# microsoft/singleshotpose

Hardware: AMD Instinct MI355X
Metric: images/sec (fwd+bwd) yolo-pose 416x416 bs=64/GPU (higher is better)
Workload: dtype f32; 1 GPU; cfg/yolo-pose.cfg train step (zero_grad+fwd+RegionLoss+bwd+grad all-reduce+SGD), 416x416, batch 64/GPU, random-init weights, 1 label/image; global_batch=64, parallelism=dp1

## Files before the change

### include/ssp_hip.h

```cpp
#ifndef SSP_HIP_H
#define SSP_HIP_H
#include <stdint.h>

#ifdef __cplusplus
extern "C" {
#endif

const char* ssp_last_error(void);
int ssp_abi_version(void);
int ssp_set_option(const char* name, int value);


int ssp_conv_fwd(const float* in, const float* wt, float* out, const float* bias, float* stats, int B, int H, int W,
                 int Cin, int Cout, int ldin, int ldout, int R, int accumulate, int plan, float* workspace,
                 int64_t workspace_floats, void* stream);
int ssp_conv_fwd_affine(const float* in, const float* wt, float* out, const float* scale, const float* shift,
                        float slope, int B, int H, int W, int Cin, int Cout, int ldin, int ldout, int R, int plan,
                        float* workspace, int64_t workspace_floats, void* stream);
int ssp_conv_stats_tile_m(int B, int H, int W, int Cin, int Cout, int R, int plan);
int ssp_conv_stats_tiles(int B, int H, int W, int Cin, int Cout, int R, int plan);
int64_t ssp_conv_stats_floats(int B, int H, int W, int Cin, int Cout, int R, int plan);
int ssp_conv_plan_wino_tile(int plan);
int64_t ssp_conv_wino_tiles(int B, int H, int W, int tile);
int ssp_wino_filter_transform_t(const float* w9, float* U, int rows, int K, int tile, void* stream);
// ... 73 lines not shown
                            const float* shift, const float* mean, const float* invstd, int C, int B, int H, int W,
                            float slope, int training, float* partial, int npartial, int zero_after, float* dgamma,
                            float* dbeta, float* c1, float* c2, void* stream);
int ssp_bn_act_bwd_affine(const float* x, int ldx, const float* g, int ldg, float* dx, int lddx, const float* scale,
                          const float* shift, const float* mean, const float* invstd, int C, int B, int H, int W, int pool,
                          float slope, void* stream);
int ssp_bn_bwd_finalize(float* partial, int npartial, int C, int64_t npix, int training, int zero_after, float* dgamma,
                        float* dbeta, float* c1, float* c2, void* stream);
int ssp_colsum(const float* g, int ldg, int64_t M, int C, float* out, void* stream);

int ssp_first_tile_pixels(void);
int ssp_first_groups(int B, int H, int W);
int ssp_first_fwd_stats(const float* x, const float* wt, float* stats, int B, int H, int W, void* stream);
int ssp_first_fwd_apply(const float* x, const float* wt, const float* scale, const float* shift, float slope, float* out,
                        int ldo, int B, int H, int W, void* stream);
int ssp_first_conv_raw(const float* x, const float* wt, float* raw, int ldraw, int B, int H, int W, void* stream);
int ssp_first_bwd_reduce(const float* x, const float* wt, const float* g, int ldg, const float* scale, const float* shift,
                         const float* mean, const float* invstd, float slope, float* partial, int B, int H, int W,
                         void* stream);
int ssp_first_bwd_wgrad(const float* x, const float* wt, const float* g, int ldg, const float* scale, const float* shift,
                        const float* mean, const float* invstd, const float* c1, const float* c2, float slope, float* dw,
                        float* workspace, int64_t workspace_floats, int B, int H, int W, void* stream);
int64_t ssp_first_wgrad_workspace_floats(int B, int H, int W);
int ssp_first_bwd_dgrad(const float* x, const float* wt, const float* g, int ldg, const float* scale, const float* shift,
                        const float* mean, const float* invstd, const float* c1, const float* c2, float slope, float* dx,
                        int B, int H, int W, void* stream);

int ssp_sgd_step(float* param, const float* grad, float* momentum_buf, int64_t n, float lr, float momentum,
                 float dampening, float weight_decay, int nesterov, int first_step, void* stream);
#define SSP_SGD_MAX_TUPLES 16
int ssp_sgd_step_table(float* param, const float* grad, float* momentum_buf, int64_t param_floats, int64_t grad_floats,
                       int64_t momentum_floats, const int64_t* table_dev, const int64_t* table_host, int nseg,
                       const float* hyper, int ntuple, void* stream);

int ssp_nchw_to_nhwc(const float* src, float* dst, int B, int C, int H, int W, int Cpad, int ld, void* stream);
int ssp_nhwc_to_nchw(const float* src, float* dst, int B, int C, int H, int W, int ld, void* stream);
int ssp_u8hwc_to_nhwc(const unsigned char* src, float* dst, int B, int H, int W, int C, int Cpad, int ld, void* stream);
typedef struct SspResampleDesc {
  const void* src;
  void* dst;
  const void* bounds;
  const void* kk;
  const void* img;
  const void* mask;
  const void* lut;
  int src_w, src_h, src_pitch;
// ... 82 lines not shown
```

### singleshotpose_amd/_lib.py

```python
import ctypes
import os
from ctypes import c_char_p, c_double, c_float, c_int, c_int64, c_void_p

_HERE = os.path.dirname(os.path.abspath(__file__))
LIB_PATH = os.environ.get("SSP_HIP_LIB") or os.path.join(_HERE, "libssp_hip.so")


class SspError(RuntimeError):
    pass


_lib = None

P = c_void_p
I = c_int
F = c_float
L = c_int64

_SIGS = {
    "ssp_abi_version": [],
    "ssp_set_option": [c_char_p, I],
    "ssp_conv_fwd": [P, P, P, P, P, I, I, I, I, I, I, I, I, I, I, P, L, P],
    "ssp_conv_fwd_affine": [P, P, P, P, P, F, I, I, I, I, I, I, I, I, I, P, L, P],
    "ssp_conv_stats_tile_m": [I, I, I, I, I, I, I],
# ... 21 lines not shown
    "ssp_conv_wgrad": [P, P, P, I, I, I, I, I, I, I, I, P],
    "ssp_conv_wgrad_route": [I, I, I, I, I, I, I, I],
    "ssp_conv_wgrad_wino": [P, P, P, I, I, I, I, I, I, I, P, L, P],
    "ssp_conv_wgrad_wino_workspace_floats": [I, I, I, I, I],
    "ssp_conv_wgrad_wino_t": [P, P, P, I, I, I, I, I, I, I, I, P, L, P],
    "ssp_conv_wgrad_wino_workspace_floats_t": [I, I, I, I, I, I],
    "ssp_bn_fwd_finalize": [P, I, I, I, I, P, P, P, P, F, F, P, P, P, P, P],
    "ssp_bn_eval_prepare": [I, P, P, P, P, F, P, P, P, P, P],
    "ssp_bn_act_fwd": [P, I, P, I, P, P, I, I, I, I, I, F, P],
    "ssp_bn_bwd_blocks": [],
    "ssp_bn_act_bwd": [P, I, P, I, P, I, P, P, P, P, I, I, I, I, I, F, I, P, P, P, P, P, P],
    "ssp_bn_act_bwd_affine": [P, I, P, I, P, I, P, P, P, P, I, I, I, I, I, F, P],
    "ssp_bn_bwd_finalize": [P, I, I, L, I, I, P, P, P, P, P],
    "ssp_first_tile_pixels": [],
    "ssp_first_groups": [I, I, I],
    "ssp_first_fwd_stats": [P, P, P, I, I, I, P],
    "ssp_first_fwd_apply": [P, P, P, P, F, P, I, I, I, I, P],
    "ssp_first_conv_raw": [P, P, P, I, I, I, I, P],
    "ssp_first_bwd_reduce": [P, P, P, I, P, P, P, P, F, P, I, I, I, P],
    "ssp_first_bwd_wgrad": [P, P, P, I, P, P, P, P, P, P, F, P, P, L, I, I, I, P],
    "ssp_first_bwd_dgrad": [P, P, P, I, P, P, P, P, P, P, F, P, I, I, I, P],
    "ssp_wino_input_transform_t": [P, I, P, I, I, I, I, I, P],
    "ssp_first_wgrad_workspace_floats": [I, I, I],
    "ssp_colsum": [P, I, L, I, P, P],
    "ssp_pose_errors": [P, I, P, P, P, I, I, P, P],
    "ssp_pts_diameter": [P, I, P, P, P],
    "ssp_pose_errors_models": [P, P, P, I, P, P, P, I, I, P, P],
    "ssp_adds_workspace_doubles": [I, I],
    "ssp_adds_errors": [P, P, P, I, I, P, P, I, P, P, L, P],
    "ssp_sgd_step": [P, P, P, L, F, F, F, F, I, I, P],
    "ssp_sgd_step_table": [P, P, P, L, L, L, P, P, I, P, I, P],
    "ssp_nchw_to_nhwc": [P, P, I, I, I, I, I, I, P],
    "ssp_nhwc_to_nchw": [P, P, I, I, I, I, I, P],
    "ssp_u8hwc_to_nhwc": [P, P, I, I, I, I, I, I, P],
    "ssp_resample_u8": [P, I, I, I, I, P],
    "ssp_distort_u8": [P, P, L, P, I, P],
    "ssp_composite_u8": [P, I, L, P],
    "ssp_repack_fwd": [P, P, I, I, I, I, P],
    "ssp_repack_dgrad": [P, P, I, I, I, I, P],
    "ssp_repack_dgrad_packed": [P, P, I, I, I, I, P],
    "ssp_unpack_grad": [P, P, I, I, I, I, P],
    "ssp_reorg": [P, I, P, I, I, I, I, I, I, I, P],
    "ssp_copy_channels": [P, I, P, I, I, L, I, P],
    "ssp_maxpool_fwd": [P, I, P, I, I, I, I, I, P],
    "ssp_maxpool_bwd": [P, I, P, I, P, I, I, I, I, I, I, P],
    "ssp_maxpool_s1_fwd": [P, I, P, I, I, I, I, I, P],
# ... 87 lines not shown
```

### singleshotpose_amd/csrc/conv_first.hip

```cpp
#include "ssp_common.h"

typedef unsigned int u32x2 __attribute__((ext_vector_type(2)));

#define FIRST_OOB 0x80000000u
constexpr int FIRST_COUT = 32;
constexpr int FIRST_BLOCK_PIX = 32;

struct FirstArgs {
  const float* x;
  const float* wt;
  int B, H, W, Ho, Wo, nxb, nblocks, bpw;
  SspFastDiv div_nxb, div_Ho;
  const float* scale; const float* shift; const float* mean; const float* invstd; const float* c1; const float* c2;
  float slope;
  float* out; int ldo;
  const float* g; int ldg;
  float* stats;
  float* dw;
  float* wpart;
};

struct FirstBlock {
  int b, yo, xb;
  bool border;
};

__device__ __forceinline__ FirstBlock first_decode(const FirstArgs& p, int blk) {
  FirstBlock k;
  const unsigned t = ssp_div((unsigned)blk, p.div_nxb);
  k.xb = blk - (int)t * p.nxb;
  const unsigned bb = ssp_div(t, p.div_Ho);
  k.yo = (int)(t - bb * (unsigned)p.Ho);
  k.b = (int)bb;
  k.border = (k.yo == 0) | (k.yo == p.Ho - 1) | (k.xb == 0) | (k.xb == p.nxb - 1);
  return k;
}

__device__ __forceinline__ void first_load(const FirstArgs& p, const __amdgpu_buffer_rsrc_t& rs, const FirstBlock& k,
                                           int lane_pix_off , int h, int pp, int q,
                                           u32x2 (&xa)[9]) {
#if defined(__HIP_DEVICE_COMPILE__)
  const int base_pix = (k.b * p.H + 2 * k.yo) * p.W + 16 * k.xb;
  if (!k.border) {
    const unsigned voff = (unsigned)(lane_pix_off * 16 + h * 8);
    const int sbase = __builtin_amdgcn_readfirstlane(base_pix) * 16;
#pragma unroll
    for (int t = 0; t < 9; ++t) {
      const int soff = sbase + ((t / 3 - 1) * p.W + (t % 3 - 1)) * 16;
      xa[t] = __builtin_amdgcn_raw_buffer_load_b64(rs, voff, soff, 0);
    }
  } else {
    const int y = 2 * k.yo + (q >> 1), x = 16 * k.xb + 2 * pp + (q & 1);
#pragma unroll
    for (int t = 0; t < 9; ++t) {
      const int yy = y + t / 3 - 1, xx = x + t % 3 - 1;
      const bool ok = ((unsigned)yy < (unsigned)p.H) && ((unsigned)xx < (unsigned)p.W);
      const unsigned voff = ok ? (unsigned)((((k.b * p.H + yy) * p.W + xx) * 4 + h * 2) * 4) : FIRST_OOB;
      xa[t] = __builtin_amdgcn_raw_buffer_load_b64(rs, voff, 0, 0);
    }
  }
#endif
}

__device__ __forceinline__ f32x16 first_conv(const u32x2 (&xa)[9], const float (&wreg)[18]) {
  f32x16 acc;
#pragma unroll
  for (int r = 0; r < 16; ++r) acc[r] = 0.f;
#pragma unroll
  for (int t = 0; t < 9; ++t) {
    const unsigned u0 = xa[t][0], u1 = xa[t][1];
    acc = __builtin_amdgcn_mfma_f32_32x32x2f32(__builtin_bit_cast(float, u0), wreg[2 * t], acc, 0, 0, 0);
    acc = __builtin_amdgcn_mfma_f32_32x32x2f32(__builtin_bit_cast(float, u1), wreg[2 * t + 1], acc, 0, 0, 0);
  }
  return acc;
}

__device__ __forceinline__ void first_load_weights(const FirstArgs& p, int cout, int h, float (&wreg)[18]) {
#pragma unroll
  for (int t = 0; t < 9; ++t) {
    wreg[2 * t] = p.wt[cout * 36 + t * 4 + 2 * h];
    wreg[2 * t + 1] = p.wt[cout * 36 + t * 4 + 2 * h + 1];
  }
}

__device__ __forceinline__ void chan_combine_f(float& n, float& mean, float& m2, float nb, float mb, float m2b) {
  const float nt = n + nb;
  if (nt > 0.f) {
    const float d = mb - mean, f = nb / nt;
    mean += d * f;
    m2 += m2b + d * d * n * f;
    n = nt;
  }
}

template <int MODE>
__global__ void __launch_bounds__(256, 3) first_block_kernel(FirstArgs p) {
#if defined(__HIP_DEVICE_COMPILE__)
  const int tid = threadIdx.x, lane = tid & 63;
  const int wid = __builtin_amdgcn_readfirstlane(tid >> 6);
  const int li = lane & 31, lh = lane >> 5;
  const int pp = li & 7, q = li >> 3;
  const int cout = li;
  const int lane_pix_off = (q >> 1) * p.W + 2 * pp + (q & 1);
  const __amdgpu_buffer_rsrc_t rs_x = __builtin_amdgcn_make_buffer_rsrc((void*)p.x, 0, (int)FIRST_OOB, 0x00020000);
  float wreg[18];
  first_load_weights(p, cout, lh, wreg);

  const int blk0 = (blockIdx.x * 4 + wid) * p.bpw;
  const int nblk = min(p.bpw, p.nblocks - blk0);

  float sc = 0.f, sh = 0.f, mu = 0.f, is = 0.f, k1 = 0.f, k2 = 0.f;
  if (MODE >= 1) { sc = p.scale[cout]; sh = p.shift[cout]; }
  if (MODE >= 2) { mu = p.mean[cout]; is = p.invstd[cout]; }
  if (MODE == 3) { k1 = p.c1[cout]; k2 = p.c2[cout]; }

  float st_n = 0.f, st_mean = 0.f, st_m2 = 0.f;
  double s1 = 0.0, s2 = 0.0;
  f32x16 accw, acct;
#pragma unroll
  for (int r = 0; r < 16; ++r) { accw[r] = 0.f; acct[r] = 0.f; }
  const int jt = li / 3, jc = li - jt * 3;
  const int w_lane_off = ((jt / 3) * p.W + (jt % 3) + 8 * lh) * 16 + jc * 4;
  const __amdgpu_buffer_rsrc_t rs_xs = __builtin_amdgcn_make_buffer_rsrc((void*)(p.x - (int64_t)(p.W + 1) * 4), 0,
                                                                         (int)FIRST_OOB, 0x00020000);

  __amdgpu_buffer_rsrc_t rs_o = rs_x, rs_g = rs_x;
  if (MODE == 1 || MODE == 4) rs_o = __builtin_amdgcn_make_buffer_rsrc((void*)p.out, 0, (int)FIRST_OOB, 0x00020000);
  if (MODE >= 2) rs_g = __builtin_amdgcn_make_buffer_rsrc((void*)p.g, 0, (int)FIRST_OOB, 0x00020000);

  auto fetch = [&](const FirstBlock& k, u32x2 (&xa)[9], float (&gv)[4]) {
    first_load(p, rs_x, k, lane_pix_off, lh, pp, q, xa);
    if constexpr (MODE == 2 || MODE == 3) {
      const int pooled_u = __builtin_amdgcn_readfirstlane((k.b * p.Ho + k.yo) * p.Wo + 8 * k.xb);
#pragma unroll
      for (int c = 0; c < 4; ++c)
        gv[c] = __builtin_bit_cast(float, __builtin_amdgcn_raw_buffer_load_b32(rs_g, (unsigned)((4 * lh * p.ldg + cout) * 4),
                                                                                (pooled_u + c) * p.ldg * 4, 0));
    }
  };
  auto compute = [&](const FirstBlock& k, const FirstBlock& kn, const u32x2 (&xa)[9], const float (&gv)[4], u32x2 (&xn)[9],
                     float (&gn)[4]) {
    float bv[16];
    if constexpr (MODE == 3) {
      const int base_pix = __builtin_amdgcn_readfirstlane((k.b * p.H + 2 * k.yo) * p.W + 16 * k.xb);
      if (!k.border) {
        const unsigned voff = (li < 27) ? (unsigned)w_lane_off : FIRST_OOB;
#pragma unroll
        for (int r = 0; r < 16; ++r) {
          const int c = r & 3, w = r >> 2;
          bv[r] = __builtin_bit_cast(float, __builtin_amdgcn_raw_buffer_load_b32(
              rs_xs, voff, (base_pix + (w >> 1) * p.W + (w & 1) + 2 * c) * 16, 0));
        }
      } else {
#pragma unroll
        for (int r = 0; r < 16; ++r) {
          const int c = r & 3, w = r >> 2;
          const int y = 2 * k.yo + (w >> 1) + jt / 3 - 1, x = 16 * k.xb + 2 * (c + 4 * lh) + (w & 1) + jt % 3 - 1;
          const bool ok = (li < 27) && ((unsigned)y < (unsigned)p.H) && ((unsigned)x < (unsigned)p.W);
          const unsigned voff = ok ? (unsigned)((((k.b * p.H + y) * p.W + x) * 4 + jc) * 4) : FIRST_OOB;
          bv[r] = __builtin_bit_cast(float, __builtin_amdgcn_raw_buffer_load_b32(rs_x, voff, 0, 0));
        }
      }
    }
    fetch(kn, xn, gn);
    const f32x16 acc = first_conv(xa, wreg);
    const int pooled_u = __builtin_amdgcn_readfirstlane((k.b * p.Ho + k.yo) * p.Wo + 8 * k.xb);

    if constexpr (MODE == 4) {
      const int base_pix = __builtin_amdgcn_readfirstlane((k.b * p.H + 2 * k.yo) * p.W + 16 * k.xb);
#pragma unroll
      for (int r = 0; r < 16; ++r) {
        const int c = r & 3, w = r >> 2;
        const float v = acc[r];
        __builtin_amdgcn_raw_buffer_store_b32(__builtin_bit_cast(unsigned, v), rs_o, (unsigned)((8 * lh * p.ldo + cout) * 4),
                                              (base_pix + (w >> 1) * p.W + (w & 1) + 2 * c) * p.ldo * 4, 0);
      }
    } else if constexpr (MODE == 0) {
      float sum = 0.f;
#pragma unroll
      for (int r = 0; r < 16; ++r) sum += acc[r];
      const float mb = sum * (1.f / 16.f);
      float m2b = 0.f;
#pragma unroll
      for (int r = 0; r < 16; ++r) { const float d = acc[r] - mb; m2b += d * d; }
      chan_combine_f(st_n, st_mean, st_m2, 16.f, mb, m2b);
    } else if constexpr (MODE == 1) {
#pragma unroll
      for (int c = 0; c < 4; ++c) {
// ... 22 lines not shown
          const float a = y > 0.f ? y : y * p.slope;
          if (a > best) { best = a; ybest = y; xbest = acc[c + 4 * w]; s = w; }
        }
        dyv[c] = ybest > 0.f ? gvc : gvc * p.slope;
        xh_sel[c] = (xbest - mu) * is;
        sel[c] = s;
      }
      if constexpr (MODE == 2) {
#pragma unroll
        for (int c = 0; c < 4; ++c) { s1 += (double)dyv[c]; s2 += (double)dyv[c] * (double)xh_sel[c]; }
      } else {
#pragma unroll
        for (int r = 0; r < 16; ++r) {
          const int c = r & 3, w = r >> 2;
          const float xh = (acc[r] - mu) * is;
          const float dyq = (sel[c] == w) ? dyv[c] : 0.f;
          const float dx = sc * (dyq - k1 - xh * k2);
          accw = __builtin_amdgcn_mfma_f32_32x32x2f32(dx, bv[r], accw, 0, 0, 0);
        }
      }
    }
  };

  u32x2 xa[9], xb[9];
  float ga[4], gb[4];
  const int last = blk0 + nblk - 1;
  FirstBlock ka = first_decode(p, nblk > 0 ? blk0 : 0), kb = ka;
  if (nblk > 0) fetch(ka, xa, ga);
  for (int g0 = 0; g0 < nblk; g0 += 8) {
    const int ge = min(nblk, g0 + 8);
    for (int ib = g0; ib < ge; ib += 2) {
      kb = first_decode(p, min(blk0 + ib + 1, last));
      compute(ka, kb, xa, ga, xb, gb);
      ka = first_decode(p, min(blk0 + ib + 2, last));
      if (ib + 1 < nblk) compute(kb, ka, xb, gb, xa, ga);
    }
    if constexpr (MODE == 3) {
      acct += accw;
#pragma unroll
      for (int r = 0; r < 16; ++r) accw[r] = 0.f;
    }
  }
  if constexpr (MODE == 3) accw = acct;

  __shared__ __attribute__((aligned(16))) float red[4][32][32];
  if constexpr (MODE == 0) {
    float on = __shfl_xor(st_n, 32), om = __shfl_xor(st_mean, 32), o2 = __shfl_xor(st_m2, 32);
// ... 14 lines not shown
    double* redd = reinterpret_cast<double*>(&red[0][0][0]);
    if (lh == 0) { redd[(wid * 32 + cout) * 2] = s1; redd[(wid * 32 + cout) * 2 + 1] = s2; }
    __syncthreads();
    if (tid < 32) {
      double a = 0.0, b = 0.0;
#pragma unroll
      for (int w = 0; w < 4; ++w) { a += redd[(w * 32 + tid) * 2]; b += redd[(w * 32 + tid) * 2 + 1]; }
      float* st = p.stats + ((int64_t)blockIdx.x * FIRST_COUT + tid) * 2;
      st[0] = (float)a;
      st[1] = (float)b;
    }
  } else if constexpr (MODE == 3) {
#pragma unroll
    for (int r = 0; r < 16; ++r) red[wid][(r & 3) + 8 * (r >> 2) + 4 * lh][li] = accw[r];
    __syncthreads();
    for (int e = tid; e < 32 * 27; e += 256) {
      const int co = e / 27, j = e - co * 27;
      p.wpart[(int64_t)blockIdx.x * (32 * 27) + e] = red[0][co][j] + red[1][co][j] + red[2][co][j] + red[3][co][j];
    }
  }
#endif
}

__global__ void __launch_bounds__(256) first_wgrad_finalize_kernel(const float* __restrict__ wpart, int nwg, float* __restrict__ dw) {
  const int tid = threadIdx.x, el = tid & 31, sl = tid >> 5;
  const int e = blockIdx.x * 32 + el;
  double a = 0.0;
  for (int w = sl; w < nwg; w += 8) a += (double)wpart[(int64_t)w * (32 * 27) + e];
  __shared__ double red[8][32];
  red[sl][el] = a;
  __syncthreads();
  if (sl == 0) {
    double t = red[0][el];
#pragma unroll
    for (int k = 1; k < 8; ++k) t += red[k][el];
    const int co = e / 27, j = e - co * 27;
    dw[co * 36 + (j / 3) * 4 + j % 3] = (float)t;
    if (e < 32 * 9) dw[e * 4 + 3] = 0.f;
  }
}

static int first_check(const float* x, const float* wt, int B, int H, int W, const char* who) {
  SSP_CHECK_ARG(x != nullptr && wt != nullptr && B > 0 && H > 0 && W > 0, "%s: null operand or empty shape", who);
  SSP_CHECK_ARG(H % 2 == 0 && W % 16 == 0, "%s: needs even H and W a multiple of 16 (8 pooled pixels per MFMA block)", who);
  SSP_CHECK_ARG((int64_t)B * H * W * 16 < (1ll << 31), "%s: input too large for 32-bit buffer offsets", who);
  SSP_CHECK_ARG((((uintptr_t)x) & 15) == 0, "%s: x must be 16-byte aligned", who);
  return SSP_OK;
}

static FirstArgs first_args(const float* x, const float* wt, int B, int H, int W, int bpw) {
  FirstArgs a;
  memset(&a, 0, sizeof(a));
  a.x = x; a.wt = wt; a.B = B; a.H = H; a.W = W; a.Ho = H / 2; a.Wo = W / 2; a.nxb = a.Wo / 8;
  a.nblocks = B * a.Ho * a.nxb;
  a.bpw = bpw;
  a.div_nxb = ssp_fastdiv((unsigned)a.nxb);
  a.div_Ho = ssp_fastdiv((unsigned)a.Ho);
  a.slope = 1.f;
// ... 35 lines not shown
  a.out = raw; a.ldo = ldraw;
  hipLaunchKernelGGL(first_block_kernel<4>, dim3(ssp_cdiv(a.nblocks, 64)), dim3(256), 0, stream, a);
  SSP_CHECK_LAUNCH("first_conv_raw");
  return SSP_OK;
}

int ssp_first_bwd_reduce_launch(const float* x, const float* wt, const float* g, int ldg, const float* scale,
                                const float* shift, const float* mean, const float* invstd, float slope, float* partial,
                                int B, int H, int W, hipStream_t stream) {
  if (int rc = first_check(x, wt, B, H, W, "first_bwd_reduce")) return rc;
  SSP_CHECK_ARG(g != nullptr && ldg >= FIRST_COUT && (int64_t)B * (H / 2) * (W / 2) * ldg * 4 < (1ll << 31),
                "first_bwd_reduce: bad gradient (ldg >= 32, < 2 GiB)");
  FirstArgs a = first_args(x, wt, B, H, W, 16);
  a.scale = scale; a.shift = shift; a.mean = mean; a.invstd = invstd; a.slope = slope; a.g = g; a.ldg = ldg;
  a.stats = partial;
  SspProfScope prof(SSP_PROF_FIRST_BWD, stream, 0.0);
  hipLaunchKernelGGL(first_block_kernel<2>, dim3(ssp_cdiv(a.nblocks, 64)), dim3(256), 0, stream, a);
  SSP_CHECK_LAUNCH("first_bwd_reduce");
  return SSP_OK;
}

int64_t ssp_first_wgrad_workspace_floats_impl(int B, int H, int W) {
  return (int64_t)ssp_cdiv((int64_t)B * (H / 2) * (W / 16), 256) * (32 * 27);
}

int ssp_first_bwd_wgrad_launch(const float* x, const float* wt, const float* g, int ldg, const float* scale,
                               const float* shift, const float* mean, const float* invstd, const float* c1,
                               const float* c2, float slope, float* dw, float* workspace, int64_t workspace_floats, int B,
                               int H, int W, hipStream_t stream) {
  if (int rc = first_check(x, wt, B, H, W, "first_bwd_wgrad")) return rc;
  SSP_CHECK_ARG(g != nullptr && ldg >= FIRST_COUT && dw != nullptr, "first_bwd_wgrad: null gradient operand");
  SSP_CHECK_ARG(workspace != nullptr && workspace_floats >= ssp_first_wgrad_workspace_floats_impl(B, H, W),
                "first_bwd_wgrad: needs a workspace of %lld floats (ssp_first_wgrad_workspace_floats)",
                (long long)ssp_first_wgrad_workspace_floats_impl(B, H, W));
  FirstArgs a = first_args(x, wt, B, H, W, 64);
  a.scale = scale; a.shift = shift; a.mean = mean; a.invstd = invstd; a.c1 = c1; a.c2 = c2; a.slope = slope;
  a.g = g; a.ldg = ldg; a.dw = dw; a.wpart = workspace;
  SspProfScope prof(SSP_PROF_FIRST_BWD, stream, 2.0 * (double)B * H * W * FIRST_COUT * 27.0);
  const int nwg = ssp_cdiv(a.nblocks, 256);
  hipLaunchKernelGGL(first_block_kernel<3>, dim3(nwg), dim3(256), 0, stream, a);
  SSP_CHECK_LAUNCH("first_bwd_wgrad");
  hipLaunchKernelGGL(first_wgrad_finalize_kernel, dim3(27), dim3(256), 0, stream, workspace, nwg, dw);
  SSP_CHECK_LAUNCH("first_wgrad_finalize");
  return SSP_OK;
}

constexpr int DG_T = 6;
constexpr int DG_RB = DG_T + 2;
constexpr int DG_RW = 16;
constexpr int DG_ZS = 27;
constexpr int DG_TS = 33;

struct FirstDgradArgs {
  FirstArgs f;
  float* dx;
  int ntx, nty;
  SspFastDiv div_ntx, div_nty;
};

__global__ void __launch_bounds__(256, 3) first_dgrad_kernel(FirstDgradArgs d) {
#if defined(__HIP_DEVICE_COMPILE__)
  const FirstArgs& p = d.f;
  __shared__ float zs[2 * DG_RB * DG_RW * DG_ZS];
  __shared__ float ts[4][32 * DG_TS];
  const int tid = threadIdx.x, lane = tid & 63;
  const int wid = __builtin_amdgcn_readfirstlane(tid >> 6);
  const int li = lane & 31, lh = lane >> 5;
  const int pp = li & 7, q = li >> 3;
  const int cout = li;
  const int lane_pix_off = (q >> 1) * p.W + 2 * pp + (q & 1);

  const unsigned t1 = ssp_div((unsigned)blockIdx.x, d.div_ntx);
  const int tx = (int)blockIdx.x - (int)t1 * d.ntx;
  const unsigned bb = ssp_div(t1, d.div_nty);
  const int ty = (int)(t1 - bb * (unsigned)d.nty), b = (int)bb;
  const int Y0 = ty * DG_T, X0 = tx * DG_T;
  const int px0 = X0 - 1;

  float wreg[18];
  first_load_weights(p, cout, lh, wreg);
  float wz[16];
  {
    const int jt = li / 3, jc = li - 3 * (li / 3);
#pragma unroll
    for (int s = 0; s < 16; ++s) wz[s] = li < 27 ? p.wt[(2 * s + lh) * 36 + jt * 4 + jc] : 0.f;
  }
  const float sc = p.scale[cout], sh = p.shift[cout], mu = p.mean[cout], is = p.invstd[cout];
  const float k1 = p.c1[cout], k2 = p.c2[cout];
  const __amdgpu_buffer_rsrc_t rs_x = __builtin_amdgcn_make_buffer_rsrc((void*)p.x, 0, (int)FIRST_OOB, 0x00020000);
  const __amdgpu_buffer_rsrc_t rs_g = __builtin_amdgcn_make_buffer_rsrc((void*)p.g, 0, (int)FIRST_OOB, 0x00020000);

  u32x2 xa[2][9];
  float gv[2][4];
#pragma unroll
  for (int i = 0; i < 2; ++i) {
    const int yo = Y0 - 1 + 2 * wid + i;
    const bool border = (yo < 1) | (yo > p.Ho - 2) | (px0 < 1) | (px0 + 9 > p.Wo);
    if (!border) {
      const int base_pix = (b * p.H + 2 * yo) * p.W + 2 * px0;
      const unsigned voff = (unsigned)(lane_pix_off * 16 + lh * 8);
      const int sbase = __builtin_amdgcn_readfirstlane(base_pix) * 16;
#pragma unroll
      for (int t = 0; t < 9; ++t) {
        const int soff = sbase + ((t / 3 - 1) * p.W + (t % 3 - 1)) * 16;
        xa[i][t] = __builtin_amdgcn_raw_buffer_load_b64(rs_x, voff, soff, 0);
      }
      const int pooled_u = __builtin_amdgcn_readfirstlane((b * p.Ho + yo) * p.Wo + px0);
#pragma unroll
      for (int c = 0; c < 4; ++c)
        gv[i][c] = __builtin_bit_cast(float, __builtin_amdgcn_raw_buffer_load_b32(rs_g, (unsigned)((4 * lh * p.ldg + cout) * 4),
                                                                                  (pooled_u + c) * p.ldg * 4, 0));
    } else {
      const int y = 2 * yo + (q >> 1), x = 2 * px0 + 2 * pp + (q & 1);
#pragma unroll
      for (int t = 0; t < 9; ++t) {
        const int yy = y + t / 3 - 1, xx = x + t % 3 - 1;
        const bool ok = ((unsigned)yy < (unsigned)p.H) && ((unsigned)xx < (unsigned)p.W);
        const unsigned voff = ok ? (unsigned)((((b * p.H + yy) * p.W + xx) * 4 + lh * 2) * 4) : FIRST_OOB;
        xa[i][t] = __builtin_amdgcn_raw_buffer_load_b64(rs_x, voff, 0, 0);
      }
#pragma unroll
      for (int c = 0; c < 4; ++c) {
        const int xo = px0 + 4 * lh + c;
        const bool ok = ((unsigned)yo < (unsigned)p.Ho) && ((unsigned)xo < (unsigned)p.Wo);
        const unsigned voff = ok ? (unsigned)((((b * p.Ho + yo) * p.Wo + xo) * p.ldg + cout) * 4) : FIRST_OOB;
        gv[i][c] = __builtin_bit_cast(float, __builtin_amdgcn_raw_buffer_load_b32(rs_g, voff, 0, 0));
      }
    }
  }

  float* slab = ts[wid];
#pragma unroll
  for (int i = 0; i < 2; ++i) {
    const int rb = 2 * wid + i, yo = Y0 - 1 + rb;
    const f32x16 acc = first_conv(xa[i], wreg);
    float dyv[4];
    int sel[4];
    bool inside[4];
#pragma unroll
    for (int c = 0; c < 4; ++c) {
      const float gvc = gv[i][c];
      float y0 = acc[c] * sc + sh;
      float best = y0 > 0.f ? y0 : y0 * p.slope, ybest = y0;
      int s = 0;
#pragma unroll
      for (int w = 1; w < 4; ++w) {
        const float y = acc[c + 4 * w] * sc + sh;
        const float a = y > 0.f ? y : y * p.slope;
        if (a > best) { best = a; ybest = y; s = w; }
      }
      dyv[c] = ybest > 0.f ? gvc : gvc * p.slope;
      sel[c] = s;
      const int xo = px0 + 4 * lh + c;
      inside[c] = ((unsigned)yo < (unsigned)p.Ho) && ((unsigned)xo < (unsigned)p.Wo);
    }
#pragma unroll
    for (int r = 0; r < 16; ++r) {
      const int c = r & 3, w = r >> 2;
// ... 70 lines not shown
```

### singleshotpose_amd/csrc/ssp_api.hip

```cpp
#include <stdarg.h>
#include <mutex>
#include <vector>

#include "../../include/ssp_hip.h"
#include "conv_wino.h"
#include "wgrad_ordered.h"
#include "conv_bf16x3.h"

int ssp_conv_tile_m(int M, int Cin, int Cout, int R, int plan);
int64_t ssp_conv_ws_floats(int M, int Cin, int Cout, int R, int plan);
int ssp_conv_igemm_launch(const float* in, const float* wt, float* out, const float* bias, float* stats, int B, int H,
                          int W, int Cin, int Cout, int ldin, int ldout, int R, int accumulate, float* ws,
                          int64_t ws_floats, int plan, int prof_kind, hipStream_t stream,
                          const float* escale = nullptr, float act_slope = 1.f, const SspBnBwdFuse* bnb = nullptr,
                          bool adj = false, const float* dM = nullptr);
int64_t ssp_wino_ws_floats(int B, int H, int W, int Cin, int Cout, int tile);
int64_t ssp_wino_adj_ws_floats(int B, int H, int W, int Cout_dy, int Cin_dx, int tile, bool own_dm);
int ssp_conv_wgrad_launch(const float* dy, const float* x, float* dw, int B, int H, int W, int Cin, int Cout, int lddy,
                          int ldx, int R, hipStream_t stream);
int64_t ssp_conv_wgrad_wino_ws_floats(int B, int H, int W, int Cin, int Cout, int tile);
int ssp_conv_s2_tile_m(int B, int H, int W, int Cout, int R);
int ssp_conv_s2_fwd_launch(const float* in, const float* wt, float* out, const float* bias, float* stats, int B, int H, int W,
                           int Cin, int Cout, int ldin, int ldout, int R, int accumulate, const float* escale,
                           float act_slope, hipStream_t stream);
// ... 22 lines not shown
                                   int C, int B, int H, int W, float slope, int training, float* partial,
                                   int npartial, int zero_after, float* dgamma, float* dbeta, float* c1, float* c2,
                                   hipStream_t stream);
int ssp_bn_act_bwd_affine_launch(const float* x, int ldx, const float* g, int ldg, float* dx, int lddx, const float* scale,
                                 const float* shift, const float* mean, const float* invstd, int C, int B, int H, int W,
                                 int pool, float slope, hipStream_t stream);
int ssp_bn_bwd_finalize_launch(float* partial, int npartial, int C, int64_t npix, int training, int zero_after,
                               float* dgamma, float* dbeta, float* c1, float* c2, hipStream_t stream);
int ssp_first_tile_pixels_impl(void);
int ssp_first_groups_impl(int B, int H, int W);
int ssp_first_fwd_stats_launch(const float* x, const float* wt, float* stats, int B, int H, int W, hipStream_t stream);
int ssp_first_fwd_apply_launch(const float* x, const float* wt, const float* scale, const float* shift, float slope,
                               float* out, int ldo, int B, int H, int W, hipStream_t stream);
int ssp_first_conv_raw_launch(const float* x, const float* wt, float* raw, int ldraw, int B, int H, int W,
                              hipStream_t stream);
int ssp_first_bwd_reduce_launch(const float* x, const float* wt, const float* g, int ldg, const float* scale,
                                const float* shift, const float* mean, const float* invstd, float slope, float* partial,
                                int B, int H, int W, hipStream_t stream);
int ssp_first_bwd_wgrad_launch(const float* x, const float* wt, const float* g, int ldg, const float* scale,
                               const float* shift, const float* mean, const float* invstd, const float* c1,
                               const float* c2, float slope, float* dw, float* workspace, int64_t workspace_floats, int B,
                               int H, int W, hipStream_t stream);
int64_t ssp_first_wgrad_workspace_floats_impl(int B, int H, int W);
int ssp_first_bwd_dgrad_launch(const float* x, const float* wt, const float* g, int ldg, const float* scale,
                               const float* shift, const float* mean, const float* invstd, const float* c1,
                               const float* c2, float slope, float* dx, int B, int H, int W, hipStream_t stream);
int ssp_colsum_launch(const float* g, int ldg, int64_t M, int C, float* out, hipStream_t stream);
int ssp_sgd_step_launch(float* p, const float* g, float* m, int64_t n, float lr, float momentum, float dampening,
                        float weight_decay, int nesterov, int first_step, hipStream_t stream);
int ssp_sgd_step_table_launch(float* p, const float* g, float* m, int64_t p_floats, int64_t g_floats, int64_t m_floats,
                              const int64_t* table_dev, const int64_t* table_host, int nseg, const float* hyper, int ntuple,
                              hipStream_t stream);
int ssp_nchw_to_nhwc_launch(const float* src, float* dst, int B, int C, int H, int W, int Cp, int ld, hipStream_t stream);
int ssp_nhwc_to_nchw_launch(const float* src, float* dst, int B, int C, int H, int W, int ld, hipStream_t stream);
int ssp_pose_errors_launch(const double* verts, int N, const double* Rt_gt, const double* Rt_pr, const double* K,
                           int k_per_pose, int n, double* out, hipStream_t stream);
int ssp_pts_diameter_launch(const double* pts, int N, double* out, double* scratch, hipStream_t stream);
int ssp_pose_errors_models_launch(const double* verts, const int* model_off, const int* pose_model, int nM,
                                  const double* Rt_gt, const double* Rt_pr, const double* K, int k_per_pose, int n,
                                  double* out, hipStream_t stream);
int64_t ssp_adds_workspace_doubles_impl(int n, int maxN);
int ssp_adds_errors_launch(const double* verts, const int* model_off, const int* pose_model, int nM, int maxN,
                           const double* Rt_gt, const double* Rt_pr, int n, double* out, double* workspace,
                           int64_t workspace_doubles, hipStream_t stream);
int ssp_resample_u8_launch(const SspResampleDesc* descs, int count, int pass, int epilogue, int max_dst_pixels, hipStream_t stream);
int ssp_distort_u8_launch(const unsigned char* rgb, unsigned char* out, int64_t npix, const unsigned char* lut, int mode, hipStream_t stream);
// ... 286 lines not shown
int ssp_first_fwd_stats(const float* x, const float* wt, float* stats, int B, int H, int W, void* stream) {
  return ssp_first_fwd_stats_launch(x, wt, stats, B, H, W, (hipStream_t)stream);
}
int ssp_first_fwd_apply(const float* x, const float* wt, const float* scale, const float* shift, float slope, float* out,
                        int ldo, int B, int H, int W, void* stream) {
  return ssp_first_fwd_apply_launch(x, wt, scale, shift, slope, out, ldo, B, H, W, (hipStream_t)stream);
}
int ssp_first_conv_raw(const float* x, const float* wt, float* raw, int ldraw, int B, int H, int W, void* stream) {
  return ssp_first_conv_raw_launch(x, wt, raw, ldraw, B, H, W, (hipStream_t)stream);
}
int ssp_first_bwd_reduce(const float* x, const float* wt, const float* g, int ldg, const float* scale, const float* shift,
                         const float* mean, const float* invstd, float slope, float* partial, int B, int H, int W,
                         void* stream) {
  return ssp_first_bwd_reduce_launch(x, wt, g, ldg, scale, shift, mean, invstd, slope, partial, B, H, W,
                                     (hipStream_t)stream);
}
int ssp_first_bwd_wgrad(const float* x, const float* wt, const float* g, int ldg, const float* scale, const float* shift,
                        const float* mean, const float* invstd, const float* c1, const float* c2, float slope, float* dw,
                        float* workspace, int64_t workspace_floats, int B, int H, int W, void* stream) {
  return ssp_first_bwd_wgrad_launch(x, wt, g, ldg, scale, shift, mean, invstd, c1, c2, slope, dw, workspace,
                                    workspace_floats, B, H, W, (hipStream_t)stream);
}
int64_t ssp_first_wgrad_workspace_floats(int B, int H, int W) { return ssp_first_wgrad_workspace_floats_impl(B, H, W); }
int ssp_first_bwd_dgrad(const float* x, const float* wt, const float* g, int ldg, const float* scale, const float* shift,
                        const float* mean, const float* invstd, const float* c1, const float* c2, float slope, float* dx,
                        int B, int H, int W, void* stream) {
  return ssp_first_bwd_dgrad_launch(x, wt, g, ldg, scale, shift, mean, invstd, c1, c2, slope, dx, B, H, W,
                                    (hipStream_t)stream);
}

int ssp_conv_wgrad(const float* dy, const float* x, float* dw, int B, int H, int W, int Cin, int Cout, int lddy,
                   int ldx, int R, void* stream) {
  return ssp_conv_wgrad_launch(dy, x, dw, B, H, W, Cin, Cout, lddy, ldx, R, (hipStream_t)stream);
}

int ssp_conv_wgrad_ordered_split(int B, int H, int W, int Cin, int Cout, int lddy, int ldx, int R, int stride, int split) {
  return ssp_wgrad_ordered_plan(B, H, W, Cin, Cout, lddy, ldx, R, stride, split).nsplit;
}
int64_t ssp_conv_wgrad_ordered_workspace_floats(int B, int H, int W, int Cin, int Cout, int lddy, int ldx, int R, int stride,
                                                int split) {
  const SspWgradOrderedPlan pl = ssp_wgrad_ordered_plan(B, H, W, Cin, Cout, lddy, ldx, R, stride, split);
  return (int64_t)pl.nsplit * pl.slab_floats;
}
int ssp_conv_wgrad_ordered(const float* dy, const float* x, float* dw, int B, int H, int W, int Cin, int Cout, int lddy, int ldx,
                           int R, int stride, int split, int flags, float* workspace, int64_t workspace_floats, void* stream) {
  SSP_CHECK_ARG(stride == 1 || stride == 2, "wgrad (ordered): stride must be 1 or 2 (got %d)", stride);
// ... 249 lines not shown
```

Before: 2641 images/s.

## Pack first-layer 3x3x3 conv K dimension to skip padded channel MFMAs

The first conv previously ran 18 MFMA 32x32x2 steps over 9 taps times 4 padded channels, wasting the zero fourth channel. A static slot table now packs the 27 real taps into 14 K-steps: the upper lane half loads full pixels for the last two taps and selects operands per step, cutting MFMAs per block by about a quarter at the cost of two extra loads and select instructions. Separately, the wgrad finalize kernel is reshaped to 16 elements by 32 slices per block, giving more reduction parallelism over workgroup partials.

After: 2650 images/s (median of 6 runs). Within noise of the previous version (+0.3%).

```diff
diff --git a/include/ssp_hip.h b/include/ssp_hip.h
--- a/include/ssp_hip.h
+++ b/include/ssp_hip.h
@@ -119,6 +119,7 @@
                         const float* mean, const float* invstd, const float* c1, const float* c2, float slope, float* dw,
                         float* workspace, int64_t workspace_floats, int B, int H, int W, void* stream);
 int64_t ssp_first_wgrad_workspace_floats(int B, int H, int W);
+int ssp_first_kslot(int step, int half);
 int ssp_first_bwd_dgrad(const float* x, const float* wt, const float* g, int ldg, const float* scale, const float* shift,
                         const float* mean, const float* invstd, const float* c1, const float* c2, float slope, float* dx,
                         int B, int H, int W, void* stream);
diff --git a/singleshotpose_amd/_lib.py b/singleshotpose_amd/_lib.py
--- a/singleshotpose_amd/_lib.py
+++ b/singleshotpose_amd/_lib.py
@@ -67,6 +67,7 @@
     "ssp_first_bwd_dgrad": [P, P, P, I, P, P, P, P, P, P, F, P, I, I, I, P],
     "ssp_wino_input_transform_t": [P, I, P, I, I, I, I, I, P],
     "ssp_first_wgrad_workspace_floats": [I, I, I],
+    "ssp_first_kslot": [I, I],
     "ssp_colsum": [P, I, L, I, P, P],
     "ssp_pose_errors": [P, I, P, P, P, I, I, P, P],
     "ssp_pts_diameter": [P, I, P, P, P],
diff --git a/singleshotpose_amd/csrc/conv_first.hip b/singleshotpose_amd/csrc/conv_first.hip
--- a/singleshotpose_amd/csrc/conv_first.hip
+++ b/singleshotpose_amd/csrc/conv_first.hip
@@ -1,10 +1,38 @@
 #include "ssp_common.h"
+#include <utility>
 
 typedef unsigned int u32x2 __attribute__((ext_vector_type(2)));
 
 #define FIRST_OOB 0x80000000u
 constexpr int FIRST_COUT = 32;
 constexpr int FIRST_BLOCK_PIX = 32;
+constexpr int FIRST_KSTEPS = 14;
+constexpr int FIRST_NLOAD = 11;
+
+constexpr int first_kslot(int s, int h) {
+  constexpr signed char FIRST_KSLOT[FIRST_KSTEPS][2] = {
+      {0 * 4 + 0, 0 * 4 + 2}, {0 * 4 + 1, 7 * 4 + 0}, {1 * 4 + 0, 1 * 4 + 2}, {1 * 4 + 1, 7 * 4 + 1},
+      {2 * 4 + 0, 2 * 4 + 2}, {2 * 4 + 1, 7 * 4 + 2}, {3 * 4 + 0, 3 * 4 + 2}, {3 * 4 + 1, 8 * 4 + 0},
+      {4 * 4 + 0, 4 * 4 + 2}, {4 * 4 + 1, 8 * 4 + 1}, {5 * 4 + 0, 5 * 4 + 2}, {5 * 4 + 1, 8 * 4 + 2},
+      {6 * 4 + 0, 6 * 4 + 2}, {6 * 4 + 1, -1}};
+  return FIRST_KSLOT[s][h];
+}
+constexpr int first_kreg(int slot, int h) {
+  if (slot < 0) return -1;
+  const int tap = slot >> 2, c = slot & 3;
+  if (tap < 7) return (c >> 1) == h ? tap * 2 + (c & 1) : -2;
+  return h == 1 ? 14 + (tap - 7) * 4 + c : -2;
+}
+constexpr bool first_ktable_ok() {
+  for (int s = 0; s < FIRST_KSTEPS; ++s)
+    for (int h = 0; h < 2; ++h) {
+      const int slot = first_kslot(s, h), reg = first_kreg(slot, h);
+      if (reg == -2 || (slot >= 0 && (slot & 3) == 3)) return false;
+      if (h == 0 && reg < 0) return false;
+    }
+  return true;
+}
+static_assert(first_ktable_ok(), "FIRST_KSLOT names a value its lane half does not load");
 
 struct FirstArgs {
   const float* x;
@@ -36,50 +64,80 @@
   return k;
 }
 
-__device__ __forceinline__ void first_load(const FirstArgs& p, const __amdgpu_buffer_rsrc_t& rs, const FirstBlock& k,
-                                           int lane_pix_off , int h, int pp, int q,
-                                           u32x2 (&xa)[9]) {
+__device__ __forceinline__ void first_load(const FirstArgs& p, const __amdgpu_buffer_rsrc_t& rs, int b, int y0, int x0,
+                                           bool border, int lane_pix_off , int h, int pp, int q,
+                                           u32x2 (&xa)[FIRST_NLOAD]) {
 #if defined(__HIP_DEVICE_COMPILE__)
-  const int base_pix = (k.b * p.H + 2 * k.yo) * p.W + 16 * k.xb;
-  if (!k.border) {
+  const int base_pix = (b * p.H + y0) * p.W + x0;
+  if (!border) {
     const unsigned voff = (unsigned)(lane_pix_off * 16 + h * 8);
+    const unsigned voff_h1 = h ? (unsigned)(lane_pix_off * 16) : FIRST_OOB;
     const int sbase = __builtin_amdgcn_readfirstlane(base_pix) * 16;
 #pragma unroll
     for (int t = 0; t < 9; ++t) {
       const int soff = sbase + ((t / 3 - 1) * p.W + (t % 3 - 1)) * 16;
-      xa[t] = __builtin_amdgcn_raw_buffer_load_b64(rs, voff, soff, 0);
+      if (t < 7) {
+        xa[t] = __builtin_amdgcn_raw_buffer_load_b64(rs, voff, soff, 0);
+      } else {
+        xa[7 + 2 * (t - 7)] = __builtin_amdgcn_raw_buffer_load_b64(rs, voff_h1, soff, 0);
+        xa[8 + 2 * (t - 7)] = __builtin_amdgcn_raw_buffer_load_b64(rs, voff_h1, soff + 8, 0);
+      }
     }
   } else {
-    const int y = 2 * k.yo + (q >> 1), x = 16 * k.xb + 2 * pp + (q & 1);
+    const int y = y0 + (q >> 1), x = x0 + 2 * pp + (q & 1);
 #pragma unroll
     for (int t = 0; t < 9; ++t) {
       const int yy = y + t / 3 - 1, xx = x + t % 3 - 1;
       const bool ok = ((unsigned)yy < (unsigned)p.H) && ((unsigned)xx < (unsigned)p.W);
-      const unsigned voff = ok ? (unsigned)((((k.b * p.H + yy) * p.W + xx) * 4 + h * 2) * 4) : FIRST_OOB;
-      xa[t] = __builtin_amdgcn_raw_buffer_load_b64(rs, voff, 0, 0);
+      const unsigned pix_off = (unsigned)(((b * p.H + yy) * p.W + xx) * 16);
+      if (t < 7) {
+        xa[t] = __builtin_amdgcn_raw_buffer_load_b64(rs, ok ? pix_off + (unsigned)(h * 8) : FIRST_OOB, 0, 0);
+      } else {
+        const unsigned voff = (ok && h) ? pix_off : FIRST_OOB;
+        xa[7 + 2 * (t - 7)] = __builtin_amdgcn_raw_buffer_load_b64(rs, voff, 0, 0);
+        xa[8 + 2 * (t - 7)] = __builtin_amdgcn_raw_buffer_load_b64(rs, voff, 8, 0);
+      }
     }
   }
 #endif
 }
 
-__device__ __forceinline__ f32x16 first_conv(const u32x2 (&xa)[9], const float (&wreg)[18]) {
+template <int S>
+__device__ __forceinline__ float first_operand(const u32x2 (&xa)[FIRST_NLOAD], bool upper) {
+  constexpr int r0 = first_kreg(first_kslot(S, 0), 0), r1 = first_kreg(first_kslot(S, 1), 1);
+  const unsigned u0 = xa[r0 >> 1][r0 & 1];
+  if constexpr (r1 == r0) {
+    return __builtin_bit_cast(float, u0);
+  } else if constexpr (r1 < 0) {
+    const unsigned u = upper ? 0u : u0;
+    return __builtin_bit_cast(float, u);
+  } else {
+    const unsigned u1 = xa[r1 >> 1][r1 & 1];
+    const unsigned u = upper ? u1 : u0;
+    return __builtin_bit_cast(float, u);
+  }
+}
+
+template <int... S>
+__device__ __forceinline__ f32x16 first_conv_steps(const u32x2 (&xa)[FIRST_NLOAD], const float (&wreg)[FIRST_KSTEPS], bool upper,
+                                                   std::integer_sequence<int, S...>) {
   f32x16 acc;
 #pragma unroll
   for (int r = 0; r < 16; ++r) acc[r] = 0.f;
-#pragma unroll
-  for (int t = 0; t < 9; ++t) {
-    const unsigned u0 = xa[t][0], u1 = xa[t][1];
-    acc = __builtin_amdgcn_mfma_f32_32x32x2f32(__builtin_bit_cast(float, u0), wreg[2 * t], acc, 0, 0, 0);
-    acc = __builtin_amdgcn_mfma_f32_32x32x2f32(__builtin_bit_cast(float, u1), wreg[2 * t + 1], acc, 0, 0, 0);
-  }
+  ((acc = __builtin_amdgcn_mfma_f32_32x32x2f32(first_operand<S>(xa, upper), wreg[S], acc, 0, 0, 0)), ...);
   return acc;
 }
 
-__device__ __forceinline__ void first_load_weights(const FirstArgs& p, int cout, int h, float (&wreg)[18]) {
-#pragma unroll
-  for (int t = 0; t < 9; ++t) {
-    wreg[2 * t] = p.wt[cout * 36 + t * 4 + 2 * h];
-    wreg[2 * t + 1] = p.wt[cout * 36 + t * 4 + 2 * h + 1];
+__device__ __forceinline__ f32x16 first_conv(const u32x2 (&xa)[FIRST_NLOAD], const float (&wreg)[FIRST_KSTEPS], int h) {
+  return first_conv_steps(xa, wreg, h != 0, std::make_integer_sequence<int, FIRST_KSTEPS>{});
+}
+
+__device__ __forceinline__ void first_load_weights(const FirstArgs& p, int cout, int h, float (&wreg)[FIRST_KSTEPS]) {
+#pragma unroll
+  for (int s = 0; s < FIRST_KSTEPS; ++s) {
+    const int s0 = first_kslot(s, 0), s1 = first_kslot(s, 1);
+    const float w = p.wt[cout * 36 + (h ? (s1 < 0 ? 0 : s1) : s0)];
+    wreg[s] = (h && s1 < 0) ? 0.f : w;
   }
 }
 
@@ -103,7 +161,7 @@
   const int cout = li;
   const int lane_pix_off = (q >> 1) * p.W + 2 * pp + (q & 1);
   const __amdgpu_buffer_rsrc_t rs_x = __builtin_amdgcn_make_buffer_rsrc((void*)p.x, 0, (int)FIRST_OOB, 0x00020000);
-  float wreg[18];
+  float wreg[FIRST_KSTEPS];
   first_load_weights(p, cout, lh, wreg);
 
   const int blk0 = (blockIdx.x * 4 + wid) * p.bpw;
@@ -128,8 +186,8 @@
   if (MODE == 1 || MODE == 4) rs_o = __builtin_amdgcn_make_buffer_rsrc((void*)p.out, 0, (int)FIRST_OOB, 0x00020000);
   if (MODE >= 2) rs_g = __builtin_amdgcn_make_buffer_rsrc((void*)p.g, 0, (int)FIRST_OOB, 0x00020000);
 
-  auto fetch = [&](const FirstBlock& k, u32x2 (&xa)[9], float (&gv)[4]) {
-    first_load(p, rs_x, k, lane_pix_off, lh, pp, q, xa);
+  auto fetch = [&](const FirstBlock& k, u32x2 (&xa)[FIRST_NLOAD], float (&gv)[4]) {
+    first_load(p, rs_x, k.b, 2 * k.yo, 16 * k.xb, k.border, lane_pix_off, lh, pp, q, xa);
     if constexpr (MODE == 2 || MODE == 3) {
       const int pooled_u = __builtin_amdgcn_readfirstlane((k.b * p.Ho + k.yo) * p.Wo + 8 * k.xb);
 #pragma unroll
@@ -138,7 +196,7 @@
                                                                                 (pooled_u + c) * p.ldg * 4, 0));
     }
   };
-  auto compute = [&](const FirstBlock& k, const FirstBlock& kn, const u32x2 (&xa)[9], const float (&gv)[4], u32x2 (&xn)[9],
+  auto compute = [&](const FirstBlock& k, const FirstBlock& kn, const u32x2 (&xa)[FIRST_NLOAD], const float (&gv)[4], u32x2 (&xn)[FIRST_NLOAD],
                      float (&gn)[4]) {
     float bv[16];
     if constexpr (MODE == 3) {
@@ -163,7 +221,7 @@
       }
     }
     fetch(kn, xn, gn);
-    const f32x16 acc = first_conv(xa, wreg);
+    const f32x16 acc = first_conv(xa, wreg, lh);
     const int pooled_u = __builtin_amdgcn_readfirstlane((k.b * p.Ho + k.yo) * p.Wo + 8 * k.xb);
 
     if constexpr (MODE == 4) {
@@ -232,7 +290,7 @@
     }
   };
 
-  u32x2 xa[9], xb[9];
+  u32x2 xa[FIRST_NLOAD], xb[FIRST_NLOAD];
   float ga[4], gb[4];
   const int last = blk0 + nblk - 1;
   FirstBlock ka = first_decode(p, nblk > 0 ? blk0 : 0), kb = ka;
@@ -293,18 +351,20 @@
 #endif
 }
 
-__global__ void __launch_bounds__(256) first_wgrad_finalize_kernel(const float* __restrict__ wpart, int nwg, float* __restrict__ dw) {
-  const int tid = threadIdx.x, el = tid & 31, sl = tid >> 5;
-  const int e = blockIdx.x * 32 + el;
+constexpr int FIRST_FIN_EL = 16, FIRST_FIN_SL = 32;
+__global__ void __launch_bounds__(FIRST_FIN_EL * FIRST_FIN_SL) first_wgrad_finalize_kernel(const float* __restrict__ wpart, int nwg,
+                                                                                          float* __restrict__ dw) {
+  const int tid = threadIdx.x, el = tid % FIRST_FIN_EL, sl = tid / FIRST_FIN_EL;
+  const int e = blockIdx.x * FIRST_FIN_EL + el;
   double a = 0.0;
-  for (int w = sl; w < nwg; w += 8) a += (double)wpart[(int64_t)w * (32 * 27) + e];
-  __shared__ double red[8][32];
+  for (int w = sl; w < nwg; w += FIRST_FIN_SL) a += (double)wpart[(int64_t)w * (32 * 27) + e];
+  __shared__ double red[FIRST_FIN_SL][FIRST_FIN_EL];
   red[sl][el] = a;
   __syncthreads();
   if (sl == 0) {
     double t = red[0][el];
 #pragma unroll
-    for (int k = 1; k < 8; ++k) t += red[k][el];
+    for (int k = 1; k < FIRST_FIN_SL; ++k) t += red[k][el];
     const int co = e / 27, j = e - co * 27;
     dw[co * 36 + (j / 3) * 4 + j % 3] = (float)t;
     if (e < 32 * 9) dw[e * 4 + 3] = 0.f;
@@ -386,6 +446,10 @@
 
 int64_t ssp_first_wgrad_workspace_floats_impl(int B, int H, int W) {
   return (int64_t)ssp_cdiv((int64_t)B * (H / 2) * (W / 16), 256) * (32 * 27);
+}
+
+int ssp_first_kslot_impl(int step, int half) {
+  return (step >= 0 && step < FIRST_KSTEPS && (half == 0 || half == 1)) ? first_kslot(step, half) : -2;
 }
 
 int ssp_first_bwd_wgrad_launch(const float* x, const float* wt, const float* g, int ldg, const float* scale,
@@ -404,7 +468,8 @@
   const int nwg = ssp_cdiv(a.nblocks, 256);
   hipLaunchKernelGGL(first_block_kernel<3>, dim3(nwg), dim3(256), 0, stream, a);
   SSP_CHECK_LAUNCH("first_bwd_wgrad");
-  hipLaunchKernelGGL(first_wgrad_finalize_kernel, dim3(27), dim3(256), 0, stream, workspace, nwg, dw);
+  hipLaunchKernelGGL(first_wgrad_finalize_kernel, dim3(32 * 27 / FIRST_FIN_EL), dim3(FIRST_FIN_EL * FIRST_FIN_SL), 0, stream,
+                     workspace, nwg, dw);
   SSP_CHECK_LAUNCH("first_wgrad_finalize");
   return SSP_OK;
 }
@@ -441,7 +506,7 @@
   const int Y0 = ty * DG_T, X0 = tx * DG_T;
   const int px0 = X0 - 1;
 
-  float wreg[18];
+  float wreg[FIRST_KSTEPS];
   first_load_weights(p, cout, lh, wreg);
   float wz[16];
   {
@@ -454,35 +519,20 @@
   const __amdgpu_buffer_rsrc_t rs_x = __builtin_amdgcn_make_buffer_rsrc((void*)p.x, 0, (int)FIRST_OOB, 0x00020000);
   const __amdgpu_buffer_rsrc_t rs_g = __builtin_amdgcn_make_buffer_rsrc((void*)p.g, 0, (int)FIRST_OOB, 0x00020000);
 
-  u32x2 xa[2][9];
+  u32x2 xa[2][FIRST_NLOAD];
   float gv[2][4];
 #pragma unroll
   for (int i = 0; i < 2; ++i) {
     const int yo = Y0 - 1 + 2 * wid + i;
     const bool border = (yo < 1) | (yo > p.Ho - 2) | (px0 < 1) | (px0 + 9 > p.Wo);
+    first_load(p, rs_x, b, 2 * yo, 2 * px0, border, lane_pix_off, lh, pp, q, xa[i]);
     if (!border) {
-      const int base_pix = (b * p.H + 2 * yo) * p.W + 2 * px0;
-      const unsigned voff = (unsigned)(lane_pix_off * 16 + lh * 8);
-      const int sbase = __builtin_amdgcn_readfirstlane(base_pix) * 16;
-#pragma unroll
-      for (int t = 0; t < 9; ++t) {
-        const int soff = sbase + ((t / 3 - 1) * p.W + (t % 3 - 1)) * 16;
-        xa[i][t] = __builtin_amdgcn_raw_buffer_load_b64(rs_x, voff, soff, 0);
-      }
       const int pooled_u = __builtin_amdgcn_readfirstlane((b * p.Ho + yo) * p.Wo + px0);
 #pragma unroll
       for (int c = 0; c < 4; ++c)
         gv[i][c] = __builtin_bit_cast(float, __builtin_amdgcn_raw_buffer_load_b32(rs_g, (unsigned)((4 * lh * p.ldg + cout) * 4),
                                                                                   (pooled_u + c) * p.ldg * 4, 0));
     } else {
-      const int y = 2 * yo + (q >> 1), x = 2 * px0 + 2 * pp + (q & 1);
-#pragma unroll
-      for (int t = 0; t < 9; ++t) {
-        const int yy = y + t / 3 - 1, xx = x + t % 3 - 1;
-        const bool ok = ((unsigned)yy < (unsigned)p.H) && ((unsigned)xx < (unsigned)p.W);
-        const unsigned voff = ok ? (unsigned)((((b * p.H + yy) * p.W + xx) * 4 + lh * 2) * 4) : FIRST_OOB;
-        xa[i][t] = __builtin_amdgcn_raw_buffer_load_b64(rs_x, voff, 0, 0);
-      }
 #pragma unroll
       for (int c = 0; c < 4; ++c) {
         const int xo = px0 + 4 * lh + c;
@@ -497,7 +547,7 @@
 #pragma unroll
   for (int i = 0; i < 2; ++i) {
     const int rb = 2 * wid + i, yo = Y0 - 1 + rb;
-    const f32x16 acc = first_conv(xa[i], wreg);
+    const f32x16 acc = first_conv(xa[i], wreg, lh);
     float dyv[4];
     int sel[4];
     bool inside[4];
diff --git a/singleshotpose_amd/csrc/ssp_api.hip b/singleshotpose_amd/csrc/ssp_api.hip
--- a/singleshotpose_amd/csrc/ssp_api.hip
+++ b/singleshotpose_amd/csrc/ssp_api.hip
@@ -68,6 +68,7 @@
                                const float* c2, float slope, float* dw, float* workspace, int64_t workspace_floats, int B,
                                int H, int W, hipStream_t stream);
 int64_t ssp_first_wgrad_workspace_floats_impl(int B, int H, int W);
+int ssp_first_kslot_impl(int step, int half);
 int ssp_first_bwd_dgrad_launch(const float* x, const float* wt, const float* g, int ldg, const float* scale,
                                const float* shift, const float* mean, const float* invstd, const float* c1,
                                const float* c2, float slope, float* dx, int B, int H, int W, hipStream_t stream);
@@ -400,6 +401,7 @@
                                     workspace_floats, B, H, W, (hipStream_t)stream);
 }
 int64_t ssp_first_wgrad_workspace_floats(int B, int H, int W) { return ssp_first_wgrad_workspace_floats_impl(B, H, W); }
+int ssp_first_kslot(int step, int half) { return ssp_first_kslot_impl(step, half); }
 int ssp_first_bwd_dgrad(const float* x, const float* wt, const float* g, int ldg, const float* scale, const float* shift,
                         const float* mean, const float* invstd, const float* c1, const float* c2, float slope, float* dx,
                         int B, int H, int W, void* stream) {
```
